# CartoonSegmentation/CartoonSegmentation

Hardware: AMD Instinct MI355X
Metric: frames/sec at 1024x1024 (seg+depth+warp) (higher is better)
Workload: dtype f32; 1 GPU; seg(RTMDet-Ins-L det640 + maskhead + ISNet refine@720, 2 instances) + LeReS depth@640 + 1 warp, frame 1024x1024; frames_per_gpu_step=8, global_batch=8, weights=closed-form synthetic (no checkpoints offline), precision=fp32 exact (v_mfma_f32_32x32x2_f32)

## Files before the change

cartoonsegmentation_amd/_lib.py:

```python
import ctypes
import os
import re

_HERE = os.path.dirname(os.path.abspath(__file__))
LIB_PATH = os.environ.get("CSM_LIB") or os.path.join(_HERE, "libcsm355.so")
HEADER_PATH = os.path.join(os.path.dirname(_HERE), "include", "csm355.h")
_lib = None


class CsmError(RuntimeError):
    pass


def declared_symbols():
    txt = open(HEADER_PATH).read()
    txt = re.sub(r"/\*.*?\*/", "", txt, flags=re.S)
    return sorted(set(re.findall(r"\b(csm_[a-z0-9_]+)\s*\(", txt)))


def load():
    global _lib
    if _lib is None:
        if not os.path.exists(LIB_PATH):
            raise CsmError("libcsm355.so not built (%s); run `python -c 'import __graft_entry__ as g; g.build()'` "
                           "or `make -C cartoonsegmentation_amd/csrc`" % LIB_PATH)
        if os.environ.get("CSM_LIB"):
            import sys
            print("libcsm355: CSM_LIB overrides the in-tree library: %s" % LIB_PATH, file=sys.stderr)
        _lib = ctypes.CDLL(LIB_PATH)
        _lib.csm_last_error.restype = ctypes.c_char_p
        _lib.csm_build_info.restype = ctypes.c_char_p
        _lib.csm_warp_frame_scratch_floats.restype = ctypes.c_size_t
        _lib.csm_fill_disocclusion_scratch_bytes.restype = ctypes.c_size_t
        _lib.csm_nms_scratch_bytes.restype = ctypes.c_size_t
        _lib.csm_autozoom_scratch_floats.restype = ctypes.c_size_t
        _lib.csm_autozoom_band_scratch_bytes.restype = ctypes.c_size_t
        _lib.csm_warp_tile_scratch_bytes.restype = ctypes.c_size_t
        _lib.csm_warp_tile_header_bytes.restype = ctypes.c_size_t
        _lib.csm_warp_frames_scratch_bytes.restype = ctypes.c_size_t
        _lib.csm_percentile_scratch_bytes.restype = ctypes.c_size_t
        _lib.csm_bokeh_depth_scratch_bytes.restype = ctypes.c_size_t
        _lib.csm_kenburns_frame_scratch_bytes.restype = ctypes.c_size_t
        _lib.csm_det_decode_scratch_bytes.restype = ctypes.c_size_t
        _lib.csm_mean_std_scratch_bytes.restype = ctypes.c_size_t
        _lib.csm_mask_rle_scratch_bytes.restype = ctypes.c_size_t
        _lib.csm_patchmatch_scratch_bytes.restype = ctypes.c_size_t
        _lib.csm_jpeg_scratch_bytes.restype = ctypes.c_size_t
        _lib.csm_png_scratch_bytes.restype = ctypes.c_size_t
        _lib.csm_jpeg_decode_scratch_bytes.restype = ctypes.c_size_t
# ... 34 lines not shown
```

cartoonsegmentation_amd/anime_instances.py:

```python
from typing import List

import numpy as np
import torch

class Colors:
    _HEX = ('FF1010', '10FF10', 'FFF010', '100FFF', '0018EC', 'FF3838', 'FF9D97', 'FF701F', 'FFB21D', 'CFD231', '48F90A', '92CC17',
            '3DDB86', '1A9334', '00D4BB', '2C99A8', '00C2FF', '344593', '6473FF', '0018EC', '8438FF', '520085', 'CB38FF', 'FF95C8',
            'FF37C7')

    def __init__(self):
        self.palette = [tuple(int(h[i:i + 2], 16) for i in (0, 2, 4)) for h in self._HEX]
        self.n = len(self.palette)

    def __call__(self, i, bgr=True):
        r, g, b = self.palette[int(i) % self.n]
        return (b, g, r) if bgr else (r, g, b)


colors = Colors()


def get_color(idx):
    return 255 if idx == -1 else colors(idx)

# ... 57 lines not shown
        mask, bbox, score = self.masks[ins_idx], self.bboxes[ins_idx], self.scores[ins_idx]
        if out_type == 'numpy' and not self.is_numpy:
            mask, bbox, score = mask.cpu().numpy(), bbox.cpu().numpy(), score.cpu().numpy()
        if out_type == 'tensor' and not self.is_tensor:
            mask, bbox, score = torch.from_numpy(mask), torch.from_numpy(bbox), torch.from_numpy(np.asarray(score))
        if isinstance(mask, torch.Tensor) and device is not None:
            mask, bbox, score = mask.to(device), bbox.to(device), score.to(device)
        return {'mask': mask, 'tags': self.tags[ins_idx], 'character_tags': self.character_tags[ins_idx], 'bbox': bbox,
                'score': score}

    def resize(self, h, w, mode='area'):
        if self.is_empty or not self.is_tensor:
            return
        oh, ow = int(self.masks.shape[1]), int(self.masks.shape[2])
        hs, ws = h / oh, w / ow
        bboxes = self.bboxes.float()
        bboxes[:, ::2] *= hs
        bboxes[:, 1::2] *= ws
        self.bboxes = torch.round(bboxes).int()
        if (oh, ow) == (h, w):
            self.masks = self.masks.to(torch.float) > 0.3
        elif self.masks.is_cuda and mode == 'area' and self.masks.dtype == torch.bool:
            from . import _lib
            from ._lib import check, f32, i32, ptr, stream_ptr
            src = self.masks.contiguous().view(torch.uint8)
            out = torch.empty((src.shape[0], h, w), dtype=torch.uint8, device=src.device)
            check(_lib.load().csm_mask_area_resize_threshold(ptr(src), i32(src.shape[0]), i32(oh), i32(ow), i32(h), i32(w), f32(0.3), ptr(out),
                                                             stream_ptr(src.device)), "mask_area_resize")
            self.masks = out.view(torch.bool)
        else:
            self.masks = torch.nn.functional.interpolate(self.masks.to(torch.float).unsqueeze(1), (h, w), mode=mode).squeeze(1) > 0.3

    def compose_masks(self, output_type=None):
        if self.is_empty:
            return None
        mask = self.masks[0]
# ... 51 lines not shown
```

cartoonsegmentation_amd/csrc/maskhead.hip:

```cpp
#include "csm_common.h"
#include "csm_resample.h"

namespace {

using csmimg::csm_sigmoid;
using csmimg::cv_src;

__device__ __forceinline__ void src_index(int dst, int in_size, int out_size, float scale, bool align, int &i0, int &i1,
                                          float &l0, float &l1) {
    if (in_size == out_size) { i0 = i1 = dst; l0 = 1.0f; l1 = 0.0f; return; }
    float real;
    if (align) real = scale * (float)dst;
    else { real = scale * ((float)dst + 0.5f) - 0.5f; if (real < 0.0f) real = 0.0f; }
    i0 = min((int)real, in_size - 1);
    i1 = i0 + (i0 < in_size - 1 ? 1 : 0);
    l1 = fminf(fmaxf(real - (float)i0, 0.0f), 1.0f);
    l0 = 1.0f - l1;
}

__global__ __launch_bounds__(64) void k_nms_mask(const float *__restrict__ boxes, const float *__restrict__ cls_off,
                                                  int n, float thr, unsigned long long *__restrict__ mask, int words) {
    int i = blockIdx.x, w = blockIdx.y, j = w * 64 + threadIdx.x;
    float ax1 = boxes[i * 4], ay1 = boxes[i * 4 + 1], ax2 = boxes[i * 4 + 2], ay2 = boxes[i * 4 + 3];
    float ao = cls_off ? cls_off[i] : 0.0f;
    ax1 += ao; ay1 += ao; ax2 += ao; ay2 += ao;
    bool sup = false;
    if (j < n && j > i) {
        float bo = cls_off ? cls_off[j] : 0.0f;
        float bx1 = boxes[j * 4] + bo, by1 = boxes[j * 4 + 1] + bo, bx2 = boxes[j * 4 + 2] + bo, by2 = boxes[j * 4 + 3] + bo;
        float left = fmaxf(ax1, bx1), right = fminf(ax2, bx2), top = fmaxf(ay1, by1), bottom = fminf(ay2, by2);
        float width = fmaxf(right - left, 0.0f), height = fmaxf(bottom - top, 0.0f);
        float inter = width * height;
        float sa = (ax2 - ax1) * (ay2 - ay1), sb = (bx2 - bx1) * (by2 - by1);
        sup = inter > thr * (sa + sb - inter);
    }
    unsigned long long b = __ballot(sup);
    if (threadIdx.x == 0) mask[(int64_t)i * words + w] = b;
}

__global__ __launch_bounds__(64) void k_nms_scan(const unsigned long long *__restrict__ mask, int n, int words,
                                                  int *__restrict__ keep, int *__restrict__ n_keep, int max_keep) {
    unsigned long long removed = 0ull;
    int lane = threadIdx.x, cnt = 0;
    for (int i = 0; i < n && cnt < max_keep; ++i) {
        unsigned long long wv = __shfl(removed, i >> 6);
        bool dead = (wv >> (i & 63)) & 1ull;
        if (!dead) {
            if (lane == 0 && cnt < max_keep) keep[cnt] = i;
            ++cnt;
            if (lane < words) removed |= mask[(int64_t)i * words + lane];
        }
    }
    if (lane == 0) *n_keep = cnt < max_keep ? cnt : max_keep;
}

template <int P, int D>
__global__ __launch_bounds__(256) void k_maskhead(const float *__restrict__ feat, int ld, int h, int w,
                                                   const float *__restrict__ params, int G,
                                                   const float *__restrict__ priors, int feat_stride,
                                                   float *__restrict__ logits) {
    __shared__ float sp[(P + 2) * D + D * D + D + D + D + 1];
    const int inst = blockIdx.y;
    for (int i = threadIdx.x; i < G; i += 256) sp[i] = params[(int64_t)inst * G + i];
    __syncthreads();
    int pix = blockIdx.x * 256 + threadIdx.x;
    if (pix >= h * w) return;
    int y = pix / w, x = pix - y * w;
    const float px = priors[inst * 4], py = priors[inst * 4 + 1], ps = priors[inst * 4 + 2];
    float in[P + 2];
    float den = ps * 8.0f;
    in[0] = (px - (float)(x * feat_stride)) / den;
    in[1] = (py - (float)(y * feat_stride)) / den;
    const float *F = feat + (int64_t)pix * ld;
#pragma unroll
    for (int c = 0; c < P; ++c) in[2 + c] = F[c];
    const float *w0 = sp, *w1 = sp + (P + 2) * D, *w2 = w1 + D * D;
    const float *b0 = w2 + D, *b1 = b0 + D, *b2 = b1 + D;
    float h0[D], h1[D];
// ... 2 lines not shown
        float a = b0[o];
#pragma unroll
        for (int c = 0; c < P + 2; ++c) a = fmaf(in[c], w0[o * (P + 2) + c], a);
        h0[o] = fmaxf(a, 0.0f);
    }
#pragma unroll
    for (int o = 0; o < D; ++o) {
        float a = b1[o];
#pragma unroll
        for (int c = 0; c < D; ++c) a = fmaf(h0[c], w1[o * D + c], a);
        h1[o] = fmaxf(a, 0.0f);
    }
    float a = b2[0];
#pragma unroll
    for (int c = 0; c < D; ++c) a = fmaf(h1[c], w2[c], a);
    logits[(int64_t)inst * h * w + pix] = a;
}

__device__ __forceinline__ float bilerp(const float *__restrict__ L, int w, int y0, int y1, int x0, int x1, float hl0,
                                        float hl1, float wl0, float wl1) {
    return hl0 * (wl0 * L[y0 * w + x0] + wl1 * L[y0 * w + x1]) + hl1 * (wl0 * L[y1 * w + x0] + wl1 * L[y1 * w + x1]);
}

__global__ __launch_bounds__(256) void k_mask_resize_threshold(const float *__restrict__ logits, int h, int w, int s,
                                                                int rh, int rw, int oh, int ow, float thr,
                                                                uint8_t *__restrict__ out) {
    const int inst = blockIdx.z;
    const int oy = blockIdx.y;
    const int ox0 = (blockIdx.x * 256 + threadIdx.x) * 4;
    if (ox0 >= ow) return;
    const float *L = logits + (int64_t)inst * h * w;
// ... 31 lines not shown
                                                           int cw, int oh, int ow, float thr, uint8_t *__restrict__ out) {
    const int inst = blockIdx.z, oy = blockIdx.y;
    const int ox = blockIdx.x * 256 + threadIdx.x;
    if (ox >= ow) return;
    const float *L = logits + (int64_t)inst * S_h * S_w;
    float sh = oh > 1 ? (float)(ch - 1) / (float)(oh - 1) : 0.0f, sw = ow > 1 ? (float)(cw - 1) / (float)(ow - 1) : 0.0f;
    int y0, y1, x0, x1; float hl0, hl1, wl0, wl1;
    src_index(oy, ch, oh, sh, true, y0, y1, hl0, hl1);
    src_index(ox, cw, ow, sw, true, x0, x1, wl0, wl1);
    float p00 = csm_sigmoid(L[y0 * S_w + x0]), p01 = csm_sigmoid(L[y0 * S_w + x1]);
    float p10 = csm_sigmoid(L[y1 * S_w + x0]), p11 = csm_sigmoid(L[y1 * S_w + x1]);
    float v = hl0 * (wl0 * p00 + wl1 * p01) + hl1 * (wl0 * p10 + wl1 * p11);
    out[((int64_t)inst * oh + oy) * ow + ox] = v > thr ? 1 : 0;
}

__global__ __launch_bounds__(256) void k_refine_batch(const uint8_t *__restrict__ img, const uint8_t *__restrict__ masks,
                                                       int H, int W, int rh, int rw, int Hm, int Wm, int rhm, int rwm, int T,
                                                       float *__restrict__ out) {
    const int inst = blockIdx.z, y = blockIdx.y, x = blockIdx.x * 256 + threadIdx.x;
    if (x >= T) return;
    float *O = out + (int64_t)inst * 4 * T * T + (int64_t)y * T + x;
    const int64_t plane = (int64_t)T * T;
    if (y >= rh || x >= rw) { O[0] = 0.0f; O[plane] = 0.0f; O[2 * plane] = 0.0f; }
    else if (rh == H && rw == W) {
        for (int c = 0; c < 3; ++c) O[c * plane] = (float)img[((int64_t)y * W + x) * 3 + c] / 255.0f;
    } else {
        double sy = (double)H / rh, sx = (double)W / rw;
        int y0, y1, x0, x1; float fy, fx;
        cv_src(y, H, sy, y0, y1, fy); cv_src(x, W, sx, x0, x1, fx);
        const int a0 = (int)rintf((1.0f - fx) * 2048.0f), a1 = (int)rintf(fx * 2048.0f);
        const int b0 = (int)rintf((1.0f - fy) * 2048.0f), b1 = (int)rintf(fy * 2048.0f);
        for (int c = 0; c < 3; ++c) {
            int r0 = img[((int64_t)y0 * W + x0) * 3 + c] * a0 + img[((int64_t)y0 * W + x1) * 3 + c] * a1;
            int r1 = img[((int64_t)y1 * W + x0) * 3 + c] * a0 + img[((int64_t)y1 * W + x1) * 3 + c] * a1;
            int v = (((b0 * (r0 >> 4)) >> 16) + ((b1 * (r1 >> 4)) >> 16) + 2) >> 2;
            v = v < 0 ? 0 : (v > 255 ? 255 : v);
            O[c * plane] = (float)v / 255.0f;
        }
    }
    const uint8_t *M = masks + (int64_t)inst * Hm * Wm;
    if (y >= rhm || x >= rwm) { O[3 * plane] = 0.0f; return; }
    if (rhm == Hm && rwm == Wm) { O[3 * plane] = (float)M[(int64_t)y * Wm + x]; return; }
    double sy = (double)Hm / rhm, sx = (double)Wm / rwm;
    int y0, y1, x0, x1; float fy, fx;
    cv_src(y, Hm, sy, y0, y1, fy); cv_src(x, Wm, sx, x0, x1, fx);
    float m00 = M[(int64_t)y0 * Wm + x0], m01 = M[(int64_t)y0 * Wm + x1], m10 = M[(int64_t)y1 * Wm + x0], m11 = M[(int64_t)y1 * Wm + x1];
    float r0 = m00 * (1.0f - fx) + m01 * fx, r1 = m10 * (1.0f - fx) + m11 * fx;
    O[3 * plane] = r0 * (1.0f - fy) + r1 * fy;
}

struct Norm3 { float mean[3], stdv[3]; };
__global__ __launch_bounds__(256) void k_det_preprocess(const uint8_t *__restrict__ img, int H, int W, int rh, int rw,
                                                         int S_h, int S_w, Norm3 nm, float pad, float *__restrict__ out) {
    const int y = blockIdx.y, x = blockIdx.x * 256 + threadIdx.x;
    if (x >= S_w) return;
// ... 40 lines not shown
    CSM_REQUIRE(mask && out && n > 0);
    k_pack_bits<<<csm::cdiv((n + 7) >> 3, 256), 256, 0, (hipStream_t)stream>>>(mask, n, out, (((uintptr_t)mask) & 7) == 0 ? 1 : 0);
    return csm::check_launch("k_pack_bits");
}

extern "C" size_t csm_nms_scratch_bytes(int n) { return (size_t)n * ((n + 63) / 64) * 8 + 64; }

extern "C" int csm_nms(const float *boxes, const float *class_offsets, int n, float iou_thr, int max_keep, int *keep,
                       int *n_keep, void *scratch, void *stream) {
    CSM_REQUIRE(keep && n_keep && n >= 0 && n <= 4096 && max_keep > 0);
    hipStream_t st = (hipStream_t)stream;
    if (n == 0) { CSM_HIP(hipMemsetAsync(n_keep, 0, sizeof(int), st)); return CSM_OK; }
    CSM_REQUIRE(boxes && scratch);
    int words = (n + 63) / 64;
    unsigned long long *mask = (unsigned long long *)scratch;
    k_nms_mask<<<dim3(n, words), 64, 0, st>>>(boxes, class_offsets, n, iou_thr, mask, words);
    int rc = csm::check_launch("k_nms_mask"); if (rc) return rc;
    k_nms_scan<<<1, 64, 0, st>>>(mask, n, words, keep, n_keep, max_keep);
    return csm::check_launch("k_nms_scan");
}

extern "C" int csm_maskhead_logits(const float *mask_feat, int ld, int h, int w, int num_prototypes,
                                   int dyconv_channels, const float *kernels, const float *priors, int n,
                                   int feat_stride, float *logits, void *stream) {
    CSM_REQUIRE(mask_feat && logits && n >= 0 && h > 0 && w > 0);
    if (n == 0) return CSM_OK;
    CSM_REQUIRE(kernels && priors);
    if (num_prototypes != 8 || dyconv_channels != 8) return csm::fail_arg("mask head compiled for 8 prototypes x 8 dyconv channels");
    k_maskhead<8, 8><<<dim3(csm::cdiv((int64_t)h * w, 256), n), 256, 0, (hipStream_t)stream>>>(
        mask_feat, ld, h, w, kernels, 169, priors, feat_stride, logits);
    return csm::check_launch("k_maskhead");
}

extern "C" int csm_mask_resize_threshold(const float *logits, int n, int h, int w, int up, int rh, int rw, int oh, int ow,
                                         float thr, uint8_t *masks, void *stream) {
    CSM_REQUIRE(masks && n >= 0 && h > 0 && w > 0 && up > 0 && rh >= oh && rw >= ow && oh > 0 && ow > 0);
    if (n == 0) return CSM_OK;
    CSM_REQUIRE(logits);
    k_mask_resize_threshold<<<dim3(csm::cdiv((ow + 3) / 4, 256), oh, n), 256, 0, (hipStream_t)stream>>>(
        logits, h, w, up, rh, rw, oh, ow, thr, masks);
    return csm::check_launch("k_mask_resize_threshold");
}

extern "C" int csm_refine_prepare_batch(const uint8_t *img_hwc, const uint8_t *masks, int n, int H, int W, int rh, int rw,
                                        int Hm, int Wm, int rhm, int rwm, int T, float *batch, void *stream) {
    CSM_REQUIRE(img_hwc && masks && batch && n > 0 && H > 0 && W > 0 && rh <= T && rw <= T);
    CSM_REQUIRE(Hm > 0 && Wm > 0 && rhm > 0 && rwm > 0 && rhm <= T && rwm <= T && rh > 0 && rw > 0);
    k_refine_batch<<<dim3(csm::cdiv(T, 256), T, n), 256, 0, (hipStream_t)stream>>>(img_hwc, masks, H, W, rh, rw, Hm, Wm, rhm,
                                                                                     rwm, T, batch);
    return csm::check_launch("k_refine_batch");
}

extern "C" int csm_refine_threshold(const float *logits, int n, int S_h, int S_w, int crop_h, int crop_w, int oh, int ow,
                                    float thr, uint8_t *masks, void *stream) {
    CSM_REQUIRE(logits && masks && n > 0 && crop_h <= S_h && crop_w <= S_w && oh > 0 && ow > 0);
    k_refine_threshold<<<dim3(csm::cdiv(ow, 256), oh, n), 256, 0, (hipStream_t)stream>>>(logits, S_h, S_w, crop_h, crop_w,
                                                                                            oh, ow, thr, masks);
    return csm::check_launch("k_refine_threshold");
}

extern "C" int csm_det_preprocess(const uint8_t *img_hwc, int H, int W, int rh, int rw, int S_h, int S_w, const float *mean3,
                                  const float *std3, float pad_value, float *out, void *stream) {
    CSM_REQUIRE(img_hwc && out && mean3 && std3 && H > 0 && W > 0 && rh <= S_h && rw <= S_w && rh > 0 && rw > 0);
    Norm3 nm;
    for (int c = 0; c < 3; ++c) { nm.mean[c] = mean3[c]; nm.stdv[c] = std3[c]; }
// ... 5 lines not shown
```

cartoonsegmentation_amd/segmentation.py:

```python
import ctypes
import json
import math
import os
from typing import List, Union

import numpy as np
import torch

from . import _lib
from ._lib import check, f32, i32, ptr, stream_ptr
from .anime_instances import AnimeInstances
from .nets import RTMDetConfig, build_isnet, build_rtmdet
from .runtime import CompiledProgram
from .weights import StateDictWeights, SynthWeights

VALID_REFINEMETHODS = {'refinenet_isnet', 'animeseg', 'none'}
ANIMESEG_CKPT = 'models/anime-seg/isnetis.ckpt'


def rescale_size(h, w, scale):
    long_e, short_e = max(scale), min(scale)
    f = min(long_e / max(h, w), short_e / min(h, w))
    return int(h * float(f) + 0.5), int(w * float(f) + 0.5)

# ... 99 lines not shown
        self.device = torch.device(device if device != 'cuda' else 'cuda:%d' % torch.cuda.current_device())
        self.ckpt, self.default_det_size, self.mask_thr = ckpt, default_det_size, mask_thr
        self.tagger, self.tagger_path = None, tagger_path
        if ckpt is None or str(ckpt).startswith('synthetic'):
            self.cfg, self._det_ws = RTMDetConfig(), SynthWeights('rtmdet.')
        else:
            blob = torch.load(ckpt, map_location='cpu', weights_only=False)
            self.cfg = config_from_ckpt_cfg(blob['meta']['cfg'])
            self._det_ws = StateDictWeights(blob['state_dict'])
        self._det_programs, self._det_weights = {}, {}
        self._refine_programs, self._refine_weights, self._refine_ws = {}, {}, None
        self._animeseg_programs, self._animeseg_weights, self._animeseg_ws = {}, {}, None
        self.refine_method = None
        self.refine_batch = int(os.environ.get('CSM_REFINE_BATCH', '16'))
        self.det_batch = max(1, int(os.environ.get('CSM_DET_BATCH', '16')))
        self.device_decode = os.environ.get('CSM_DEVICE_DECODE', '0') == '1'
        self.set_refine_method(**(refine_kwargs or {'refine_method': 'none'}))

    def set_detect_size(self, det_size: Union[int, tuple]):
        self.default_det_size = det_size if isinstance(det_size, int) else max(det_size)

    def set_refine_method(self, refine_method: str = 'none', refine_size: int = 720, refinenet_ckpt: str = None, **kw):
        if refine_method not in VALID_REFINEMETHODS:
            raise NotImplementedError('Invalid refine method: %s' % refine_method)
        self.refine_method, self.refine_size = refine_method, refine_size
        if refine_method == 'animeseg' and self._animeseg_ws is None:
            synthetic = str(self.ckpt).startswith('synthetic') or os.environ.get('CSM_SYNTHETIC_WEIGHTS', '0') == '1'
            self._animeseg_ws = load_animeseg_weights(refinenet_ckpt, synthetic)
        if refine_method == 'refinenet_isnet' and self._refine_ws is None:
            refinenet_ckpt = refinenet_ckpt or 'models/AnimeInstanceSegmentation/refine_last.ckpt'
# ... 57 lines not shown
                imgs, return_list = find_all_imgs(imgs, abs_path=True), True
            elif imgs.endswith('.json'):
                raise NotImplementedError("COCO files are read by the annotation export only (infer(..., save_annotation=path))")
        imgs = imgs if return_list else [imgs]
        insts = self._infer_frames(imgs, pred_score_thr)
        if output_type == 'numpy':
            for inst in insts:
                inst.to_numpy()
        return insts if return_list else insts[0]

    def _infer_frames(self, imgs, pred_score_thr):
        if any(isinstance(im, str) for im in imgs):
            imgs = self._load(imgs)
        same = len(imgs) > 1 and all(tuple(im.shape) == tuple(imgs[0].shape) for im in imgs)
        if same:
            insts = [self._instances_from(d, pred_score_thr) for d in self.detect_raw_batch(imgs)]
            if self.refine_method == 'refinenet_isnet':
                self._refine_many(list(zip(insts, imgs)), self.refine_size)
            elif self.refine_method == 'animeseg':
                self._animeseg_refine(list(zip(insts, imgs)), self.refine_size)
        else:
            insts = []
            for img in imgs:
                inst = self._det_forward(img, pred_score_thr)
                if self.refine_method == 'refinenet_isnet':
                    self._postprocess_refine(inst, img, refine_size=self.refine_size)
                elif self.refine_method == 'animeseg':
                    self._animeseg_refine([(inst, img)], self.refine_size)
                insts.append(inst)
        return insts

# ... 120 lines not shown
        slots = L.csm_det_decode_slots(level_hw, i32(nl), i32(nc), i32(cfg.nms_pre))
        if slots < 0:
            raise _lib.CsmError("detector decode: nms_pre <= 1024 and at most 4096 candidates per image are supported")
        K = min(slots, 4096)
        scores = torch.empty((nb, K), dtype=torch.float32, device=dev)
        boxes = torch.empty((nb, K, 4), dtype=torch.float32, device=dev)
        src = torch.empty((nb, K), dtype=torch.int32, device=dev)
        labels = torch.empty((nb, K), dtype=torch.int32, device=dev)
        offs = torch.empty((nb, K), dtype=torch.float32, device=dev) if nc > 1 else None
        scratch = torch.empty(L.csm_det_decode_scratch_bytes(i32(nb), i32(slots)), dtype=torch.uint8, device=dev)
        sfx, sfy = float(np.float32(1 / w_scale)), float(np.float32(1 / h_scale))
        check(L.csm_det_decode(cls_p, reg_p, level_hw, strides, lds3, i32(nl), i32(nb), i32(nc), f32(cfg.score_thr), i32(cfg.nms_pre),
                               f32(rw), f32(rh), f32(sfx), f32(sfy), f32(cfg.min_bbox_size), i32(K), ptr(scores), ptr(boxes), ptr(src),
                               ptr(labels), ptr(offs), ptr(scratch), stream_ptr()), "det_decode")
        keep = torch.zeros((nb, M), dtype=torch.int32, device=dev)
        nk = torch.zeros(nb, dtype=torch.int32, device=dev)
        nscr = torch.empty(L.csm_nms_scratch_bytes(i32(K)), dtype=torch.uint8, device=dev)
        for bi in range(nb):
            check(L.csm_nms(ptr(boxes[bi]), ptr(None if offs is None else offs[bi]), i32(K), f32(cfg.nms_iou), i32(M),
                            ptr(keep[bi]), ptr(nk[bi:bi + 1]), ptr(nscr), stream_ptr()), "nms")
        k_scores = torch.empty((nb, M), dtype=torch.float32, device=dev)
        k_boxes = torch.empty((nb, M, 4), dtype=torch.float32, device=dev)
        k_labels = torch.empty((nb, M), dtype=torch.int32, device=dev)
        k_priors = torch.empty((nb, M, 4), dtype=torch.float32, device=dev)
        k_kernels = torch.empty((nb, M, G), dtype=torch.float32, device=dev)
        check(L.csm_det_gather(ker_p, level_hw, strides, lds3, i32(nl), i32(nb), i32(K), i32(M), i32(G), ptr(keep), ptr(scores), ptr(boxes),
                               ptr(src), ptr(labels), ptr(k_scores), ptr(k_boxes), ptr(k_labels), ptr(k_priors), ptr(k_kernels),
                               stream_ptr()), "det_gather")
        nk_h, ks_h = nk.tolist(), k_scores.tolist()
        outs = []
        for bi in range(nb):
            n = sum(1 for j in range(nk_h[bi]) if ks_h[bi][j] > cfg.score_thr)
            out = dict(H=H, W=W, S=S, rh=rh, rw=rw, w_scale=w_scale, h_scale=h_scale, rp=rp, cp=cp, bi=bi, n=n)
            if n:
                out.update(boxes=k_boxes[bi, :n], scores=k_scores[bi, :n], priors=k_priors[bi, :n], kernels=k_kernels[bi, :n],
                           labels=k_labels[bi, :n], scores_host=ks_h[bi][:n])
            outs.append(out)
        return outs

    def _masks_from(self, d, sel=None):
        L, cfg = _lib.load(), self.cfg
        pri, ker = (d['priors'], d['kernels']) if sel is None else (d['priors'][sel].contiguous(), d['kernels'][sel].contiguous())
        n = int(pri.shape[0])
        mf, ld, h, w = self._mask_feat_of(d)
        logits = torch.empty((n, h, w), dtype=torch.float32, device=self.device)
        check(L.csm_maskhead_logits(ptr(mf), i32(ld), i32(h), i32(w), i32(cfg.num_prototypes), i32(cfg.dyconv_channels),
                                    ptr(ker), ptr(pri), i32(n), i32(cfg.strides[0]), ptr(logits), stream_ptr()), "maskhead")
        up = cfg.strides[0]
# ... 22 lines not shown
            return AnimeInstances()
        hs = d.get('scores_host')
        if hs is not None:
            idx = [j for j, v in enumerate(hs) if np.float32(v) > np.float32(pred_score_thr)]
            if not idx:
                return AnimeInstances()
            sel = torch.tensor(idx, dtype=torch.long, device=self.device)
        else:
            sel = (d['scores'] > pred_score_thr).nonzero()[:, 0]
            if sel.numel() < 1:
                return AnimeInstances()
        masks = self._masks_from(d, sel).bool()
        bboxes = d['boxes'][sel].to(torch.int32)
        bboxes[:, 2:] -= bboxes[:, :2]
        return AnimeInstances(masks, bboxes, d['scores'][sel])

    def infer_embeddings(self, imgs, det_size=None):
        if det_size is not None:
            self.set_detect_size(det_size)
        img = imgs[0] if isinstance(imgs, list) else imgs
        d = self.detect_raw(img)
        if d['n'] == 0:
            d.update(boxes=torch.zeros((0, 4), device=self.device), scores=torch.zeros(0, device=self.device),
                     priors=torch.zeros((0, 4), device=self.device), kernels=torch.zeros((0, self.cfg.num_gen_params), device=self.device))
        d['bboxes'] = d['boxes']
        mask_feat = d['cp'].view(d['rp'].mask_feat)[d.get('bi', 0)][..., :self.cfg.num_prototypes].clone()
        d['mask_feat'] = mask_feat
        return img, d, mask_feat

    def segment_with_bboxes(self, img, bboxes, instance_data, mask_feat=None):
# ... 15 lines not shown
        ker_sel, pri_sel = d['kernels'][idx].contiguous(), d['priors'][idx].contiguous()
        check(L.csm_maskhead_logits(ptr(feat), i32(ld), i32(fh), i32(fw), i32(cfg.num_prototypes), i32(cfg.dyconv_channels),
                                    ptr(ker_sel), ptr(pri_sel), i32(n), i32(cfg.strides[0]), ptr(logits), stream_ptr()), "maskhead")
        masks = torch.empty((n, H, W), dtype=torch.uint8, device=self.device)
        check(L.csm_mask_resize_threshold(ptr(logits), i32(n), i32(fh), i32(fw), i32(cfg.strides[0]), i32(long_side),
                                          i32(long_side), i32(H), i32(W), f32(0.5), ptr(masks), stream_ptr()), "mask_resize")
        bb = t[idx].to(torch.int32)
        bb[:, 2:] -= bb[:, :2]
        inst = AnimeInstances(masks.bool(), bb, d['scores'][idx])
        if self.refine_method == 'refinenet_isnet':
            self._postprocess_refine(inst, img, refine_size=self.refine_size)
        return inst

    def _refine_many(self, pairs, refine_size=720, max_batch=None):
        L = _lib.load()
        jobs = []
        for inst, img in pairs:
            if inst.is_empty:
                continue
            img_d = self._upload(img)
            segs = inst.masks.to(self.device).to(torch.uint8).contiguous()
            jobs.append((inst, img_d, segs))
        if not jobs:
            return
        H, W = int(jobs[0][1].shape[0]), int(jobs[0][1].shape[1])
        T = refine_size
        rh, rw = scaledown_size(H, W, T)
        Hm, Wm = int(jobs[0][2].shape[1]), int(jobs[0][2].shape[2])
        rhm, rwm = scaledown_size(Hm, Wm, T)
        flat = [(j, k) for j, (_, _, segs) in enumerate(jobs) for k in range(segs.shape[0])]
        outs = [torch.empty((segs.shape[0], H, W), dtype=torch.uint8, device=self.device) for _, _, segs in jobs]
        max_batch = max_batch or self.refine_batch
        for c0 in range(0, len(flat), max_batch):
            chunk = flat[c0:c0 + max_batch]
            b = len(chunk)
            cp = self._refiner(b, T)
            batch = torch.empty((b, 4, T, T), dtype=torch.float32, device=self.device)
            for i, (j, k) in enumerate(chunk):
                check(L.csm_refine_prepare_batch(ptr(jobs[j][1]), ptr(jobs[j][2][k:k + 1]), i32(1), i32(H), i32(W), i32(rh), i32(rw),
                                                 i32(Hm), i32(Wm), i32(rhm), i32(rwm), i32(T), ptr(batch[i:i + 1]), stream_ptr()),
                      "refine_prepare")
            logits = torch.empty((b, 1, T, T), dtype=torch.float32, device=self.device)
            cp.run(batch, logits)
            for i, (j, k) in enumerate(chunk):
                check(L.csm_refine_threshold(ptr(logits[i:i + 1]), i32(1), i32(T), i32(T), i32(rh), i32(rw), i32(H), i32(W),
                                             f32(self.mask_thr), ptr(outs[j][k:k + 1]), stream_ptr()), "refine_threshold")
        for (inst, _, _), o in zip(jobs, outs):
# ... 69 lines not shown
```

include/csm355.h:

```cpp
#ifndef CSM355_H
#define CSM355_H
#include <stddef.h>
#include <stdint.h>
#ifdef __cplusplus
extern "C" {
#endif

#define CSM_OK 0
#define CSM_ERR_ARG 1
#define CSM_ERR_HIP 2
#define CSM_ERR_NAN 3
#define CSM_ERR_DATA 4

const char *csm_last_error(void);
int csm_version(void);
const char *csm_build_info(void);


int csm_pointrender_update_zee(const float *pts, int B, int64_t N, int H, int W, double focal,
                               double baseline, float *zee, void *stream);

int csm_pointrender_degrid(const float *zee_in, float *zee_out, int B, int H, int W, void *stream);

int csm_pointrender_update_output(const float *pts, const float *data, const float *zee, int B, int C,
// ... 146 lines not shown

int csm_det_decode_slots(const int *level_hw, int n_levels, int num_classes, int nms_pre);
size_t csm_det_decode_scratch_bytes(int nb, int slots);
int csm_det_decode(const float *const *cls, const float *const *reg, const int *level_hw, const int *strides, const int *lds3,
                   int n_levels, int nb, int num_classes, float score_thr, int nms_pre, float clamp_w, float clamp_h,
                   float scale_x, float scale_y, float min_bbox_size, int K, float *scores, float *boxes, int *src, int *labels,
                   float *class_offsets, void *scratch, void *stream);
int csm_det_gather(const float *const *kern, const int *level_hw, const int *strides, const int *lds3, int n_levels, int nb, int K,
                   int max_keep, int num_gen_params, const int *keep, const float *scores, const float *boxes, const int *src,
                   const int *labels, float *kept_scores, float *kept_boxes, int *kept_labels, float *kept_priors,
                   float *kept_kernels, void *stream);

size_t csm_nms_scratch_bytes(int n);
int csm_nms(const float *boxes, const float *class_offsets, int n, float iou_thr, int max_keep, int *keep,
            int *n_keep, void *scratch, void *stream);

int csm_maskhead_logits(const float *mask_feat, int ld, int h, int w, int num_prototypes, int dyconv_channels,
                        const float *kernels, const float *priors, int n, int feat_stride, float *logits,
                        void *stream);

int csm_mask_resize_threshold(const float *logits, int n, int h, int w, int up, int rh, int rw, int oh, int ow,
                              float thr, uint8_t *masks, void *stream);

int csm_refine_prepare_batch(const uint8_t *img_hwc, const uint8_t *masks, int n, int H, int W, int rh, int rw, int Hm, int Wm,
                             int rhm, int rwm, int T, float *batch, void *stream);

int csm_refine_threshold(const float *logits, int n, int S_h, int S_w, int crop_h, int crop_w, int oh, int ow, float thr,
                         uint8_t *masks, void *stream);

int csm_animeseg_prepare(const uint8_t *img_hwc, int H, int W, int h, int w, int s, int bgr_to_rgb, float *out_nchw, void *stream);

int csm_animeseg_mask(const float *logits, int s, int h, int w, int H0, int W0, float thr, float *prob_out, uint8_t *fg_out,
                      void *stream);

int csm_animeseg_select(uint8_t *masks_u8, int k, int Hm, int Wm, const uint8_t *fg, int W0, unsigned *counts_scratch,
                        void *stream);

size_t csm_mask_rle_scratch_bytes(int n, int H, int W);
int csm_mask_rle_measure(const uint8_t *masks, int n, int H, int W, int64_t *info, void *scratch, void *stream);
int csm_mask_rle_write(const uint8_t *masks, int n, int H, int W, const int64_t *info, char *out, void *scratch, void *stream);
// ... 109 lines not shown
```

Baseline: 135.4 frames/s.

## Batch segmentation glue: NMS, mask head, and refine prep across frames

Replaces per-frame NMS launches with a single batched NMS kernel, and merges the per-frame mask-head, resize-threshold and box conversion into one batched launch over all frames. Refine preparation now takes per-item image and mask pointers, so instances from several frames share one refine batch. The goal is fewer kernel launches, fewer host syncs and fewer small allocations in the glue between stages. It adds a fallback path and an environment toggle, plus host-side checks that kept indices are contiguous.

New measurement: 137.7 frames/s, median of 6. 1.7% higher.

```diff
diff --git a/cartoonsegmentation_amd/_lib.py b/cartoonsegmentation_amd/_lib.py
--- a/cartoonsegmentation_amd/_lib.py
+++ b/cartoonsegmentation_amd/_lib.py
@@ -33,6 +33,7 @@
         _lib.csm_warp_frame_scratch_floats.restype = ctypes.c_size_t
         _lib.csm_fill_disocclusion_scratch_bytes.restype = ctypes.c_size_t
         _lib.csm_nms_scratch_bytes.restype = ctypes.c_size_t
+        _lib.csm_nms_batch_scratch_bytes.restype = ctypes.c_size_t
         _lib.csm_autozoom_scratch_floats.restype = ctypes.c_size_t
         _lib.csm_autozoom_band_scratch_bytes.restype = ctypes.c_size_t
         _lib.csm_warp_tile_scratch_bytes.restype = ctypes.c_size_t
diff --git a/cartoonsegmentation_amd/anime_instances.py b/cartoonsegmentation_amd/anime_instances.py
--- a/cartoonsegmentation_amd/anime_instances.py
+++ b/cartoonsegmentation_amd/anime_instances.py
@@ -95,12 +95,14 @@
             return
         oh, ow = int(self.masks.shape[1]), int(self.masks.shape[2])
         hs, ws = h / oh, w / ow
-        bboxes = self.bboxes.float()
-        bboxes[:, ::2] *= hs
-        bboxes[:, 1::2] *= ws
-        self.bboxes = torch.round(bboxes).int()
+        if (oh, ow) != (h, w) or self.bboxes.dtype != torch.int32:
+            bboxes = self.bboxes.float()
+            bboxes[:, ::2] *= hs
+            bboxes[:, 1::2] *= ws
+            self.bboxes = torch.round(bboxes).int()
         if (oh, ow) == (h, w):
-            self.masks = self.masks.to(torch.float) > 0.3
+            if self.masks.dtype != torch.bool:
+                self.masks = self.masks.to(torch.float) > 0.3
         elif self.masks.is_cuda and mode == 'area' and self.masks.dtype == torch.bool:
             from . import _lib
             from ._lib import check, f32, i32, ptr, stream_ptr
diff --git a/cartoonsegmentation_amd/csrc/maskhead.hip b/cartoonsegmentation_amd/csrc/maskhead.hip
--- a/cartoonsegmentation_amd/csrc/maskhead.hip
+++ b/cartoonsegmentation_amd/csrc/maskhead.hip
@@ -19,8 +19,12 @@
 }
 
 __global__ __launch_bounds__(64) void k_nms_mask(const float *__restrict__ boxes, const float *__restrict__ cls_off,
-                                                  int n, float thr, unsigned long long *__restrict__ mask, int words) {
+                                                  int n, float thr, unsigned long long *__restrict__ mask, int words,
+                                                  int64_t img_words) {
     int i = blockIdx.x, w = blockIdx.y, j = w * 64 + threadIdx.x;
+    boxes += (int64_t)blockIdx.z * n * 4;
+    if (cls_off) cls_off += (int64_t)blockIdx.z * n;
+    mask += (int64_t)blockIdx.z * img_words;
     float ax1 = boxes[i * 4], ay1 = boxes[i * 4 + 1], ax2 = boxes[i * 4 + 2], ay2 = boxes[i * 4 + 3];
     float ao = cls_off ? cls_off[i] : 0.0f;
     ax1 += ao; ay1 += ao; ax2 += ao; ay2 += ao;
@@ -39,7 +43,11 @@
 }
 
 __global__ __launch_bounds__(64) void k_nms_scan(const unsigned long long *__restrict__ mask, int n, int words,
-                                                  int *__restrict__ keep, int *__restrict__ n_keep, int max_keep) {
+                                                  int *__restrict__ keep, int *__restrict__ n_keep, int max_keep,
+                                                  int64_t img_words) {
+    mask += (int64_t)blockIdx.x * img_words;
+    keep += (int64_t)blockIdx.x * max_keep;
+    n_keep += blockIdx.x;
     unsigned long long removed = 0ull;
     int lane = threadIdx.x, cnt = 0;
     for (int i = 0; i < n && cnt < max_keep; ++i) {
@@ -54,14 +62,27 @@
     if (lane == 0) *n_keep = cnt < max_keep ? cnt : max_keep;
 }
 
+constexpr int kDetChunk = 16;
+struct DetFrames { int start[kDetChunk + 1]; int nf; };
+
 template <int P, int D>
-__global__ __launch_bounds__(256) void k_maskhead(const float *__restrict__ feat, int ld, int h, int w,
+__global__ __launch_bounds__(256) void k_maskhead(const float *__restrict__ feat, int64_t feat_frame, int ld, int h, int w,
                                                    const float *__restrict__ params, int G,
-                                                   const float *__restrict__ priors, int feat_stride,
-                                                   float *__restrict__ logits) {
+                                                   const float *__restrict__ priors, int slots, int feat_stride,
+                                                   float *__restrict__ logits, const float *__restrict__ boxes,
+                                                   int *__restrict__ boxes_out, DetFrames FR) {
     __shared__ float sp[(P + 2) * D + D * D + D + D + D + 1];
-    const int inst = blockIdx.y;
-    for (int i = threadIdx.x; i < G; i += 256) sp[i] = params[(int64_t)inst * G + i];
+    const int flat = blockIdx.y;
+    int f = 0;
+    while (f + 1 < FR.nf && flat >= FR.start[f + 1]) ++f;
+    const int64_t inst = (int64_t)f * slots + (flat - FR.start[f]);
+    feat += (int64_t)f * feat_frame;
+    for (int i = threadIdx.x; i < G; i += 256) sp[i] = params[inst * G + i];
+    if (boxes_out && blockIdx.x == 0 && threadIdx.x < 4) {
+        const int t = threadIdx.x;
+        const unsigned v = (unsigned)(int)boxes[inst * 4 + t];
+        boxes_out[(int64_t)flat * 4 + t] = (int)(t < 2 ? v : v - (unsigned)(int)boxes[inst * 4 + t - 2]);
+    }
     __syncthreads();
     int pix = blockIdx.x * 256 + threadIdx.x;
     if (pix >= h * w) return;
@@ -94,7 +115,7 @@
     float a = b2[0];
 #pragma unroll
     for (int c = 0; c < D; ++c) a = fmaf(h1[c], w2[c], a);
-    logits[(int64_t)inst * h * w + pix] = a;
+    logits[(int64_t)flat * h * w + pix] = a;
 }
 
 __device__ __forceinline__ float bilerp(const float *__restrict__ L, int w, int y0, int y1, int x0, int x1, float hl0,
@@ -156,11 +177,14 @@
     out[((int64_t)inst * oh + oy) * ow + ox] = v > thr ? 1 : 0;
 }
 
-__global__ __launch_bounds__(256) void k_refine_batch(const uint8_t *__restrict__ img, const uint8_t *__restrict__ masks,
-                                                       int H, int W, int rh, int rw, int Hm, int Wm, int rhm, int rwm, int T,
-                                                       float *__restrict__ out) {
+constexpr int kRefineChunk = 16;
+struct RefineItems { const uint8_t *img[kRefineChunk]; const uint8_t *mask[kRefineChunk]; };
+
+__global__ __launch_bounds__(256) void k_refine_batch(RefineItems R, int H, int W, int rh, int rw, int Hm, int Wm, int rhm,
+                                                       int rwm, int T, float *__restrict__ out) {
     const int inst = blockIdx.z, y = blockIdx.y, x = blockIdx.x * 256 + threadIdx.x;
     if (x >= T) return;
+    const uint8_t *__restrict__ img = R.img[inst];
     float *O = out + (int64_t)inst * 4 * T * T + (int64_t)y * T + x;
     const int64_t plane = (int64_t)T * T;
     if (y >= rh || x >= rw) { O[0] = 0.0f; O[plane] = 0.0f; O[2 * plane] = 0.0f; }
@@ -180,7 +204,7 @@
             O[c * plane] = (float)v / 255.0f;
         }
     }
-    const uint8_t *M = masks + (int64_t)inst * Hm * Wm;
+    const uint8_t *__restrict__ M = R.mask[inst];
     if (y >= rhm || x >= rwm) { O[3 * plane] = 0.0f; return; }
     if (rhm == Hm && rwm == Wm) { O[3 * plane] = (float)M[(int64_t)y * Wm + x]; return; }
     double sy = (double)Hm / rhm, sx = (double)Wm / rwm;
@@ -251,9 +275,29 @@
     CSM_REQUIRE(boxes && scratch);
     int words = (n + 63) / 64;
     unsigned long long *mask = (unsigned long long *)scratch;
-    k_nms_mask<<<dim3(n, words), 64, 0, st>>>(boxes, class_offsets, n, iou_thr, mask, words);
+    k_nms_mask<<<dim3(n, words), 64, 0, st>>>(boxes, class_offsets, n, iou_thr, mask, words, 0);
     int rc = csm::check_launch("k_nms_mask"); if (rc) return rc;
-    k_nms_scan<<<1, 64, 0, st>>>(mask, n, words, keep, n_keep, max_keep);
+    k_nms_scan<<<1, 64, 0, st>>>(mask, n, words, keep, n_keep, max_keep, 0);
+    return csm::check_launch("k_nms_scan");
+}
+
+extern "C" size_t csm_nms_batch_scratch_bytes(int nb, int n) {
+    if (nb <= 0 || n < 0) return 0;
+    return (size_t)nb * csm_nms_scratch_bytes(n);
+}
+
+extern "C" int csm_nms_batch(const float *boxes, const float *class_offsets, int nb, int n, float iou_thr, int max_keep, int *keep,
+                             int *n_keep, void *scratch, void *stream) {
+    CSM_REQUIRE(keep && n_keep && nb > 0 && nb <= 65535 && n >= 0 && n <= 4096 && max_keep > 0);
+    hipStream_t st = (hipStream_t)stream;
+    if (n == 0) { CSM_HIP(hipMemsetAsync(n_keep, 0, (size_t)nb * sizeof(int), st)); return CSM_OK; }
+    CSM_REQUIRE(boxes && scratch && !(((uintptr_t)scratch) & 7));
+    const int words = (n + 63) / 64;
+    const int64_t img_words = (int64_t)(csm_nms_scratch_bytes(n) / 8);
+    unsigned long long *mask = (unsigned long long *)scratch;
+    k_nms_mask<<<dim3(n, words, nb), 64, 0, st>>>(boxes, class_offsets, n, iou_thr, mask, words, img_words);
+    int rc = csm::check_launch("k_nms_mask"); if (rc) return rc;
+    k_nms_scan<<<nb, 64, 0, st>>>(mask, n, words, keep, n_keep, max_keep, img_words);
     return csm::check_launch("k_nms_scan");
 }
 
@@ -264,8 +308,11 @@
     if (n == 0) return CSM_OK;
     CSM_REQUIRE(kernels && priors);
     if (num_prototypes != 8 || dyconv_channels != 8) return csm::fail_arg("mask head compiled for 8 prototypes x 8 dyconv channels");
+    CSM_REQUIRE(n <= 65535);
+    DetFrames F{};
+    F.nf = 1; F.start[1] = n;
     k_maskhead<8, 8><<<dim3(csm::cdiv((int64_t)h * w, 256), n), 256, 0, (hipStream_t)stream>>>(
-        mask_feat, ld, h, w, kernels, 169, priors, feat_stride, logits);
+        mask_feat, 0, ld, h, w, kernels, 169, priors, n, feat_stride, logits, nullptr, nullptr, F);
     return csm::check_launch("k_maskhead");
 }
 
@@ -279,13 +326,74 @@
     return csm::check_launch("k_mask_resize_threshold");
 }
 
+extern "C" int csm_det_masks_batch(const float *mask_feat, int64_t sample_stride, int ld, int h, int w, int num_prototypes,
+                                   int dyconv_channels, const float *kernels, const float *priors, const float *boxes, int nb,
+                                   int max_keep, const int *n_k, int feat_stride, int up, int rh, int rw, int oh, int ow, float thr,
+                                   float *logits, uint8_t *masks, int *boxes_xywh, void *stream) {
+    CSM_REQUIRE(nb > 0 && n_k && max_keep > 0 && h > 0 && w > 0 && ld >= num_prototypes && sample_stride >= 0);
+    CSM_REQUIRE(up > 0 && rh >= oh && rw >= ow && oh > 0 && ow > 0);
+    if (num_prototypes != 8 || dyconv_channels != 8) return csm::fail_arg("mask head compiled for 8 prototypes x 8 dyconv channels");
+    int64_t total = 0;
+    for (int k = 0; k < nb; ++k) { CSM_REQUIRE(n_k[k] >= 0 && n_k[k] <= max_keep); total += n_k[k]; }
+    if (total == 0) return CSM_OK;
+    CSM_REQUIRE(total <= 65535 && mask_feat && kernels && priors && boxes && logits && masks && boxes_xywh);
+    hipStream_t st = (hipStream_t)stream;
+    const int64_t hw = (int64_t)h * w;
+    int done = 0;
+    for (int f0 = 0; f0 < nb; f0 += kDetChunk) {
+        DetFrames F{};
+        F.nf = nb - f0 < kDetChunk ? nb - f0 : kDetChunk;
+        for (int k = 0; k < F.nf; ++k) F.start[k + 1] = F.start[k] + n_k[f0 + k];
+        const int n = F.start[F.nf];
+        if (n == 0) continue;
+        k_maskhead<8, 8><<<dim3(csm::cdiv(hw, 256), n), 256, 0, st>>>(
+            mask_feat + (int64_t)f0 * sample_stride, sample_stride, ld, h, w, kernels + (int64_t)f0 * max_keep * 169, 169,
+            priors + (int64_t)f0 * max_keep * 4, max_keep, feat_stride, logits + (int64_t)done * hw,
+            boxes + (int64_t)f0 * max_keep * 4, boxes_xywh + (int64_t)done * 4, F);
+        int rc = csm::check_launch("k_maskhead"); if (rc) return rc;
+        done += n;
+    }
+    k_mask_resize_threshold<<<dim3(csm::cdiv((ow + 3) / 4, 256), oh, (int)total), 256, 0, st>>>(logits, h, w, up, rh, rw, oh, ow,
+                                                                                                 thr, masks);
+    return csm::check_launch("k_mask_resize_threshold");
+}
+
+namespace {
+int refine_prepare_launch(const uint8_t *const *imgs, const uint8_t *const *masks, int n, int H, int W, int rh, int rw, int Hm,
+                          int Wm, int rhm, int rwm, int T, float *batch, hipStream_t st) {
+    for (int i0 = 0; i0 < n; i0 += kRefineChunk) {
+        RefineItems R{};
+        const int ni = n - i0 < kRefineChunk ? n - i0 : kRefineChunk;
+        for (int i = 0; i < ni; ++i) { R.img[i] = imgs[i0 + i]; R.mask[i] = masks[i0 + i]; }
+        k_refine_batch<<<dim3(csm::cdiv(T, 256), T, ni), 256, 0, st>>>(R, H, W, rh, rw, Hm, Wm, rhm, rwm, T,
+                                                                        batch + (int64_t)i0 * 4 * T * T);
+        int rc = csm::check_launch("k_refine_batch"); if (rc) return rc;
+    }
+    return CSM_OK;
+}
+}
+
 extern "C" int csm_refine_prepare_batch(const uint8_t *img_hwc, const uint8_t *masks, int n, int H, int W, int rh, int rw,
                                         int Hm, int Wm, int rhm, int rwm, int T, float *batch, void *stream) {
     CSM_REQUIRE(img_hwc && masks && batch && n > 0 && H > 0 && W > 0 && rh <= T && rw <= T);
     CSM_REQUIRE(Hm > 0 && Wm > 0 && rhm > 0 && rwm > 0 && rhm <= T && rwm <= T && rh > 0 && rw > 0);
-    k_refine_batch<<<dim3(csm::cdiv(T, 256), T, n), 256, 0, (hipStream_t)stream>>>(img_hwc, masks, H, W, rh, rw, Hm, Wm, rhm,
-                                                                                     rwm, T, batch);
-    return csm::check_launch("k_refine_batch");
+    for (int i0 = 0; i0 < n; i0 += kRefineChunk) {
+        const uint8_t *ip[kRefineChunk], *mp[kRefineChunk];
+        const int ni = n - i0 < kRefineChunk ? n - i0 : kRefineChunk;
+        for (int i = 0; i < ni; ++i) { ip[i] = img_hwc; mp[i] = masks + (int64_t)(i0 + i) * Hm * Wm; }
+        int rc = refine_prepare_launch(ip, mp, ni, H, W, rh, rw, Hm, Wm, rhm, rwm, T, batch + (int64_t)i0 * 4 * T * T,
+                                       (hipStream_t)stream);
+        if (rc) return rc;
+    }
+    return CSM_OK;
+}
+
+extern "C" int csm_refine_prepare_many(const uint8_t *const *imgs_hwc, const uint8_t *const *masks, int n, int H, int W, int rh,
+                                       int rw, int Hm, int Wm, int rhm, int rwm, int T, float *batch, void *stream) {
+    CSM_REQUIRE(imgs_hwc && masks && batch && n > 0 && H > 0 && W > 0 && rh <= T && rw <= T);
+    CSM_REQUIRE(Hm > 0 && Wm > 0 && rhm > 0 && rwm > 0 && rhm <= T && rwm <= T && rh > 0 && rw > 0);
+    for (int i = 0; i < n; ++i) CSM_REQUIRE(imgs_hwc[i] && masks[i]);
+    return refine_prepare_launch(imgs_hwc, masks, n, H, W, rh, rw, Hm, Wm, rhm, rwm, T, batch, (hipStream_t)stream);
 }
 
 extern "C" int csm_refine_threshold(const float *logits, int n, int S_h, int S_w, int crop_h, int crop_w, int oh, int ow,
diff --git a/cartoonsegmentation_amd/segmentation.py b/cartoonsegmentation_amd/segmentation.py
--- a/cartoonsegmentation_amd/segmentation.py
+++ b/cartoonsegmentation_amd/segmentation.py
@@ -137,6 +137,7 @@
         self.refine_method = None
         self.refine_batch = int(os.environ.get('CSM_REFINE_BATCH', '16'))
         self.det_batch = max(1, int(os.environ.get('CSM_DET_BATCH', '16')))
+        self.seg_glue_batch = os.environ.get('CSM_SEG_GLUE_BATCH', '1') != '0'
         self.device_decode = os.environ.get('CSM_DEVICE_DECODE', '0') == '1'
         self.set_refine_method(**(refine_kwargs or {'refine_method': 'none'}))
 
@@ -224,7 +225,10 @@
             imgs = self._load(imgs)
         same = len(imgs) > 1 and all(tuple(im.shape) == tuple(imgs[0].shape) for im in imgs)
         if same:
-            insts = [self._instances_from(d, pred_score_thr) for d in self.detect_raw_batch(imgs)]
+            dets = self.detect_raw_batch(imgs)
+            insts = self._instances_from_run(dets, pred_score_thr) if self.seg_glue_batch else None
+            if insts is None:
+                insts = [self._instances_from(d, pred_score_thr) for d in dets]
             if self.refine_method == 'refinenet_isnet':
                 self._refine_many(list(zip(insts, imgs)), self.refine_size)
             elif self.refine_method == 'animeseg':
@@ -375,12 +379,20 @@
                                f32(rw), f32(rh), f32(sfx), f32(sfy), f32(cfg.min_bbox_size), i32(K), ptr(scores), ptr(boxes), ptr(src),
                                ptr(labels), ptr(offs), ptr(scratch), stream_ptr()), "det_decode")
         keep = torch.zeros((nb, M), dtype=torch.int32, device=dev)
-        nk = torch.zeros(nb, dtype=torch.int32, device=dev)
-        nscr = torch.empty(L.csm_nms_scratch_bytes(i32(K)), dtype=torch.uint8, device=dev)
-        for bi in range(nb):
-            check(L.csm_nms(ptr(boxes[bi]), ptr(None if offs is None else offs[bi]), i32(K), f32(cfg.nms_iou), i32(M),
-                            ptr(keep[bi]), ptr(nk[bi:bi + 1]), ptr(nscr), stream_ptr()), "nms")
-        k_scores = torch.empty((nb, M), dtype=torch.float32, device=dev)
+        batched = self.seg_glue_batch
+        if batched:
+            read = torch.empty(nb * M + nb, dtype=torch.float32, device=dev)
+            k_scores, nk = read[:nb * M].view(nb, M), read[nb * M:].view(torch.int32)
+            nscr = torch.empty(L.csm_nms_batch_scratch_bytes(i32(nb), i32(K)), dtype=torch.uint8, device=dev)
+            check(L.csm_nms_batch(ptr(boxes), ptr(offs), i32(nb), i32(K), f32(cfg.nms_iou), i32(M), ptr(keep), ptr(nk), ptr(nscr),
+                                  stream_ptr()), "nms_batch")
+        else:
+            nk = torch.zeros(nb, dtype=torch.int32, device=dev)
+            nscr = torch.empty(L.csm_nms_scratch_bytes(i32(K)), dtype=torch.uint8, device=dev)
+            for bi in range(nb):
+                check(L.csm_nms(ptr(boxes[bi]), ptr(None if offs is None else offs[bi]), i32(K), f32(cfg.nms_iou), i32(M),
+                                ptr(keep[bi]), ptr(nk[bi:bi + 1]), ptr(nscr), stream_ptr()), "nms")
+            k_scores = torch.empty((nb, M), dtype=torch.float32, device=dev)
         k_boxes = torch.empty((nb, M, 4), dtype=torch.float32, device=dev)
         k_labels = torch.empty((nb, M), dtype=torch.int32, device=dev)
         k_priors = torch.empty((nb, M, 4), dtype=torch.float32, device=dev)
@@ -388,11 +400,16 @@
         check(L.csm_det_gather(ker_p, level_hw, strides, lds3, i32(nl), i32(nb), i32(K), i32(M), i32(G), ptr(keep), ptr(scores), ptr(boxes),
                                ptr(src), ptr(labels), ptr(k_scores), ptr(k_boxes), ptr(k_labels), ptr(k_priors), ptr(k_kernels),
                                stream_ptr()), "det_gather")
-        nk_h, ks_h = nk.tolist(), k_scores.tolist()
+        if batched:
+            host = read.cpu().numpy()
+            nk_h, ks_h = host[nb * M:].view(np.int32).tolist(), host[:nb * M].reshape(nb, M).tolist()
+        else:
+            nk_h, ks_h = nk.tolist(), k_scores.tolist()
+        run = dict(nb=nb, M=M, boxes=k_boxes, scores=k_scores, priors=k_priors, kernels=k_kernels)
         outs = []
         for bi in range(nb):
             n = sum(1 for j in range(nk_h[bi]) if ks_h[bi][j] > cfg.score_thr)
-            out = dict(H=H, W=W, S=S, rh=rh, rw=rw, w_scale=w_scale, h_scale=h_scale, rp=rp, cp=cp, bi=bi, n=n)
+            out = dict(H=H, W=W, S=S, rh=rh, rw=rw, w_scale=w_scale, h_scale=h_scale, rp=rp, cp=cp, bi=bi, n=n, run=run)
             if n:
                 out.update(boxes=k_boxes[bi, :n], scores=k_scores[bi, :n], priors=k_priors[bi, :n], kernels=k_kernels[bi, :n],
                            labels=k_labels[bi, :n], scores_host=ks_h[bi][:n])
@@ -445,6 +462,40 @@
         bboxes = d['boxes'][sel].to(torch.int32)
         bboxes[:, 2:] -= bboxes[:, :2]
         return AnimeInstances(masks, bboxes, d['scores'][sel])
+
+    def _instances_from_run(self, dets, pred_score_thr: float = 0.3):
+        L, cfg = _lib.load(), self.cfg
+        run = dets[0].get('run')
+        if run is None or len(dets) != run['nb'] or any(d.get('run') is not run or d['bi'] != k or 'mask_feat' in d for k, d in enumerate(dets)):
+            return None
+        n_k = []
+        for d in dets:
+            idx = [j for j, v in enumerate(d['scores_host']) if np.float32(v) > np.float32(pred_score_thr)] if d['n'] else []
+            if idx != list(range(len(idx))):
+                return None
+            n_k.append(len(idx))
+        total = sum(n_k)
+        if total == 0:
+            return [AnimeInstances() for _ in dets]
+        d0 = dets[0]
+        v = d0['rp'].mask_feat
+        b = v.buf
+        feat = d0['cp'].workspace[b.offset:]
+        h, w, up = v.h, v.w, cfg.strides[0]
+        rh2 = math.ceil(h * up * (1 / d0['w_scale'])); rw2 = math.ceil(w * up * (1 / d0['h_scale']))
+        oh, ow = min(rh2, d0['H']), min(rw2, d0['W'])
+        logits = torch.empty((total, h, w), dtype=torch.float32, device=self.device)
+        masks = torch.empty((total, oh, ow), dtype=torch.uint8, device=self.device)
+        bboxes = torch.empty((total, 4), dtype=torch.int32, device=self.device)
+        check(L.csm_det_masks_batch(ptr(feat), ctypes.c_int64(v.h * v.w * b.c), i32(b.c), i32(h), i32(w), i32(cfg.num_prototypes),
+                                    i32(cfg.dyconv_channels), ptr(run['kernels']), ptr(run['priors']), ptr(run['boxes']), i32(run['nb']),
+                                    i32(run['M']), (ctypes.c_int * len(n_k))(*n_k), i32(up), i32(up), i32(rh2), i32(rw2), i32(oh), i32(ow),
+                                    f32(cfg.mask_thr_binary), ptr(logits), ptr(masks), ptr(bboxes), stream_ptr()), "det_masks_batch")
+        insts, s = [], 0
+        for k, n in enumerate(n_k):
+            insts.append(AnimeInstances(masks[s:s + n].view(torch.bool), bboxes[s:s + n], run['scores'][k, :n]) if n else AnimeInstances())
+            s += n
+        return insts
 
     def infer_embeddings(self, imgs, det_size=None):
         if det_size is not None:
@@ -490,12 +541,17 @@
 
     def _refine_many(self, pairs, refine_size=720, max_batch=None):
         L = _lib.load()
+        batched = self.seg_glue_batch
         jobs = []
         for inst, img in pairs:
             if inst.is_empty:
                 continue
             img_d = self._upload(img)
-            segs = inst.masks.to(self.device).to(torch.uint8).contiguous()
+            segs = inst.masks.to(self.device)
+            if batched and segs.dtype == torch.bool and segs.is_contiguous():
+                segs = segs.view(torch.uint8)
+            else:
+                segs = segs.to(torch.uint8).contiguous()
             jobs.append((inst, img_d, segs))
         if not jobs:
             return
@@ -505,8 +561,29 @@
         Hm, Wm = int(jobs[0][2].shape[1]), int(jobs[0][2].shape[2])
         rhm, rwm = scaledown_size(Hm, Wm, T)
         flat = [(j, k) for j, (_, _, segs) in enumerate(jobs) for k in range(segs.shape[0])]
+        max_batch = max_batch or self.refine_batch
+        if batched:
+            block = torch.empty((len(flat), H, W), dtype=torch.uint8, device=self.device)
+            for c0 in range(0, len(flat), max_batch):
+                chunk = flat[c0:c0 + max_batch]
+                b = len(chunk)
+                cp = self._refiner(b, T)
+                batch = torch.empty((b, 4, T, T), dtype=torch.float32, device=self.device)
+                VP = ctypes.c_void_p * b
+                check(L.csm_refine_prepare_many(VP(*[jobs[j][1].data_ptr() for j, _ in chunk]),
+                                                VP(*[jobs[j][2].data_ptr() + k * Hm * Wm for j, k in chunk]), i32(b), i32(H), i32(W),
+                                                i32(rh), i32(rw), i32(Hm), i32(Wm), i32(rhm), i32(rwm), i32(T), ptr(batch), stream_ptr()),
+                      "refine_prepare_many")
+                logits = torch.empty((b, 1, T, T), dtype=torch.float32, device=self.device)
+                cp.run(batch, logits)
+                check(L.csm_refine_threshold(ptr(logits), i32(b), i32(T), i32(T), i32(rh), i32(rw), i32(H), i32(W),
+                                             f32(self.mask_thr), ptr(block[c0:c0 + b]), stream_ptr()), "refine_threshold")
+            s = 0
+            for inst, _, segs in jobs:
+                inst.masks = block[s:s + segs.shape[0]].view(torch.bool)
+                s += segs.shape[0]
+            return
         outs = [torch.empty((segs.shape[0], H, W), dtype=torch.uint8, device=self.device) for _, _, segs in jobs]
-        max_batch = max_batch or self.refine_batch
         for c0 in range(0, len(flat), max_batch):
             chunk = flat[c0:c0 + max_batch]
             b = len(chunk)
diff --git a/include/csm355.h b/include/csm355.h
--- a/include/csm355.h
+++ b/include/csm355.h
@@ -184,6 +184,9 @@
 size_t csm_nms_scratch_bytes(int n);
 int csm_nms(const float *boxes, const float *class_offsets, int n, float iou_thr, int max_keep, int *keep,
             int *n_keep, void *scratch, void *stream);
+size_t csm_nms_batch_scratch_bytes(int nb, int n);
+int csm_nms_batch(const float *boxes, const float *class_offsets, int nb, int n, float iou_thr, int max_keep, int *keep,
+                  int *n_keep, void *scratch, void *stream);
 
 int csm_maskhead_logits(const float *mask_feat, int ld, int h, int w, int num_prototypes, int dyconv_channels,
                         const float *kernels, const float *priors, int n, int feat_stride, float *logits,
@@ -191,9 +194,15 @@
 
 int csm_mask_resize_threshold(const float *logits, int n, int h, int w, int up, int rh, int rw, int oh, int ow,
                               float thr, uint8_t *masks, void *stream);
+int csm_det_masks_batch(const float *mask_feat, int64_t sample_stride, int ld, int h, int w, int num_prototypes,
+                        int dyconv_channels, const float *kernels, const float *priors, const float *boxes, int nb, int max_keep,
+                        const int *n_k, int feat_stride, int up, int rh, int rw, int oh, int ow, float thr, float *logits,
+                        uint8_t *masks, int *boxes_xywh, void *stream);
 
 int csm_refine_prepare_batch(const uint8_t *img_hwc, const uint8_t *masks, int n, int H, int W, int rh, int rw, int Hm, int Wm,
                              int rhm, int rwm, int T, float *batch, void *stream);
+int csm_refine_prepare_many(const uint8_t *const *imgs_hwc, const uint8_t *const *masks, int n, int H, int W, int rh, int rw,
+                            int Hm, int Wm, int rhm, int rwm, int T, float *batch, void *stream);
 
 int csm_refine_threshold(const float *logits, int n, int S_h, int S_w, int crop_h, int crop_w, int oh, int ow, float thr,
                          uint8_t *masks, void *stream);
```
